# tridivb/attention_based_tbn

Hardware: AMD Instinct MI355X
Metric: clips/sec (3-seg RGB+Flow+Audio TBN fwd+bwd) (higher is better)
Workload: dtype f32; 1 GPU; BASELINE config 4: RGB+Flow+Audio async, attention off, 3 segments, 224x224 frames + 1.279 s (256x256) spectrogram, train step fwd+loss+bwd+clip+SGD; batch_per_gpu=32, global_batch=32, segments=3, parallelism=single, launch_plans=committed (bench_plans.json)

## Files before the change

attention_based_tbn_amd/_lib.py:

```python
import ctypes as C
import os

_HERE = os.path.dirname(os.path.abspath(__file__))
LIB_PATH = os.path.join(_HERE, "libtbn_hip.so")
if os.environ.get("TBN_LIB"):
    import sys as _sys
    LIB_PATH = os.path.abspath(os.environ["TBN_LIB"])
    print(f"[tbn] TBN_LIB set: loading {LIB_PATH} instead of the shipped libtbn_hip.so", file=_sys.stderr)

c_fp = C.c_void_p
c_i = C.c_int
c_sz = C.c_size_t
c_f = C.c_float


class ConvInfo(C.Structure):
    _fields_ = [("name", C.c_char * 64), ("cin", c_i), ("cout", c_i), ("ksize", c_i), ("stride", c_i),
                ("pad", c_i), ("weight_offset", c_sz), ("channel_offset", c_sz)]


class BackboneParams(C.Structure):
    _fields_ = [("weight", c_fp), ("bias", c_fp), ("gamma", c_fp), ("beta", c_fp), ("running_mean", c_fp),
                ("running_var", c_fp), ("momentum", c_f), ("eps", c_f), ("side_stream", c_fp), ("flags", c_i),
                ("weight_planes", c_fp)]
# ... 95 lines not shown
    "tbn_stem_conv_wgrad": (c_i, [c_fp, c_i, c_fp, c_fp] + [c_i] * 8 + [c_fp, c_fp]),
    "tbn_linear_fwd": (c_i, [c_fp, c_i, c_fp, c_fp, c_fp, c_i, c_i, c_i, c_i, c_i, c_fp]),
    "tbn_linear_dgrad": (c_i, [c_fp, c_i, c_fp, c_fp, c_i, c_i, c_i, c_i, c_i, c_fp, c_fp]),
    "tbn_linear_wgrad_workspace_floats": (c_sz, [c_i, c_i, c_i]),
    "tbn_linear_wgrad": (c_i, [c_fp, c_i, c_fp, c_i, c_fp, c_fp, c_i, c_i, c_i, c_fp, c_fp]),
    "tbn_bn_workspace_floats": (c_sz, [c_i, c_i]),
    "tbn_bn_relu_train_fwd": (c_i, [c_fp, c_i, c_i, c_fp, c_fp, c_fp, c_fp, c_f, c_f, c_fp, c_fp, c_fp, c_fp, c_fp,
                                    c_i, c_fp, c_fp]),
    "tbn_bn_relu_train_bwd": (c_i, [c_fp, c_i, c_fp, c_i, c_i, c_fp, c_fp, c_fp, c_fp, c_fp, c_fp, c_fp, c_fp, c_fp]),
    "tbn_bn_stats_partials": (c_i, [c_fp, c_i, c_i, c_i, c_fp, C.POINTER(c_i), c_fp]),
    "tbn_bn_fwd_batch": (c_i, [C.POINTER(BnFwdDesc), c_i, c_f, c_f, c_fp]),
    "tbn_bn_bwd_partial_floats": (c_sz, [c_i, c_i]),
    "tbn_bn_bwd_batch": (c_i, [C.POINTER(BnBwdDesc), c_i, c_fp]),
    "tbn_bn_relu_maxpool_train_fwd": (c_i, [c_fp, c_i, c_i, c_i, c_i, c_fp, c_fp, c_fp, c_fp, c_f, c_f, c_fp, c_fp, c_fp,
                                            c_fp, c_fp, c_i, c_fp, c_i, c_i, c_i, c_i, c_fp, c_fp]),
    "tbn_bn_relu_maxpool_train_bwd": (c_i, [c_fp, c_i, c_fp, c_fp, c_i, c_i, c_i, c_i, c_i, c_i, c_i, c_i, c_fp, c_fp,
                                            c_fp, c_fp, c_fp, c_fp, c_fp, c_fp, c_fp]),
    "tbn_bn_res_apply": (c_i, [c_fp, c_i, c_i, c_i, c_fp, c_fp, c_fp, c_i, c_i, c_fp, c_i, c_fp]),
    "tbn_bn_res_fwd": (c_i, [c_fp, c_i, c_i, c_i, c_fp, c_i, c_i, c_fp, c_fp, c_fp, c_fp, c_f, c_f, c_fp, c_fp, c_fp,
                             c_fp, c_fp, c_i, c_i, c_fp, c_i, c_fp]),
    "tbn_bn_res_bwd_workspace_floats": (c_sz, [c_i, c_i]),
    "tbn_bn_res_bwd": (c_i, [c_fp, c_i, c_fp, c_i, c_fp, c_i, c_i, c_i, c_fp, c_fp, c_fp, c_i, c_fp, c_i, c_fp, c_i, c_i,
                             c_fp, c_fp, c_fp, c_fp]),
    "tbn_maxpool3_fwd": (c_i, [c_fp, c_i, c_fp, c_i, c_fp] + [c_i] * 8 + [c_fp]),
    "tbn_maxpool3_bwd": (c_i, [c_fp, c_i, c_fp, c_fp, c_i] + [c_i] * 9 + [c_fp]),
    "tbn_avgpool3_fwd": (c_i, [c_fp, c_i, c_fp, c_i] + [c_i] * 5 + [c_fp]),
    "tbn_spatial_mean_fwd": (c_i, [c_fp, c_i, c_fp, c_i] + [c_i] * 5 + [c_fp]),
    "tbn_spatial_mean_bwd": (c_i, [c_fp, c_i, c_fp, c_i] + [c_i] * 5 + [c_fp]),
    "tbn_pe_concat_fwd": (c_i, [c_fp, c_i, c_fp, c_fp, c_i, c_i, c_i, c_i, c_i, c_fp]),
    "tbn_groupnorm_fwd": (c_i, [c_fp, c_fp, c_fp, c_fp, c_fp, c_fp, c_i, c_i, c_i, c_i, c_f, c_fp]),
# ... 94 lines not shown
```

attention_based_tbn_amd/core/models/bn_inception.py:

```python
import ctypes as C
import os
import weakref
from collections import OrderedDict

import torch
import torch.nn as nn

from ... import _lib
from ..._lib import BUCKET_CB, BackboneGrads, BackboneParams, ConvInfo, TbnHipError, call, lib, ptr, stream_ptr
from ... import ops

_BLOCKS = [("3a", True, True), ("3b", True, True), ("3c", False, False), ("4a", True, True), ("4b", True, True),
           ("4c", True, True), ("4d", True, True), ("4e", False, False), ("5a", True, True), ("5b", True, True)]


def reference_conv_order():
    names = ["conv1_7x7_s2", "conv2_3x3_reduce", "conv2_3x3"]
    for b, has1, hasp in _BLOCKS:
        p = "inception_" + b
        if has1:
            names.append(p + "_1x1")
        names += [p + "_3x3_reduce", p + "_3x3", p + "_double_3x3_reduce", p + "_double_3x3_1", p + "_double_3x3_2"]
        if hasp:
            names.append(p + "_pool_proj")
# ... 224 lines not shown
    def __init__(self, num_classes=1000, in_channels=3):
        super().__init__()
        self.in_channels = in_channels
        self.num_classes = num_classes
        self.is_audio = False
        self.attend = False
        self.feature_size = 1024
        self.eval_chunk = 256
        self.autotune = True
        self.use_aux_stream = True
        self._aux_streams = {}
        self.use_branch_streams = True
        self._side_streams = {}
        self.use_riders = True
        self.stem_wgrad_last = False
        self._conv_math = "f32"
        self._conv_math_layers = "3x3"
        self._planes = None
        self._planes_key = None
        self._last_flip = None
        self._out_slot = None
        self.plan_sync = None
        self.grad_bucket_fn = None
        self._plans = OrderedDict()
        probe = C.c_void_p()
        call("tbn_backbone_plan_create", in_channels, 1, 64, 64, C.byref(probe))
        self._layers = OrderedDict()
        info = ConvInfo()
        for i in range(lib().tbn_backbone_num_convs(probe)):
            call("tbn_backbone_conv_info", probe, i, C.byref(info))
# ... 108 lines not shown
        return self._plans[key]

    def plan_fingerprints(self):
        return {k: p.fingerprint() for k, p in self._plans.items()}

    def flip_weights_early(self):
        f = self._last_flip() if getattr(self, "_last_flip", None) is not None else None
        self._last_flip = None
        if f is None or f.done or f.weight._version != f.version or torch.cuda.is_current_stream_capturing():
            return False
        prm = BackboneParams(ptr(f.weight), 0, 0, 0, 0, 0, 0.1, 1e-5, 0, 0)
        call("tbn_backbone_flip_weights", f.plan.handle, C.byref(prm), ptr(f.ws), f.ws.numel(), stream_ptr())
        f.done = True
        return True

    CONV_MATH = {"f32": 0, "bf16x6": 8, "bf16x3": 16}

    @property
    def conv_math(self):
        return self._conv_math

    @conv_math.setter
    def conv_math(self, value):
        if value not in self.CONV_MATH:
            raise ValueError("conv_math must be one of %s, got %r" % (", ".join(map(repr, self.CONV_MATH)), value))
        self._conv_math = value
        if value == "f32":
            self._planes = self._planes_key = None

    CONV_MATH_LAYERS = ("3x3", "all")
# ... 18 lines not shown
        w = self.flat_weight
        np_ = 6 if self._conv_math == "bf16x6" else 3
        key = (w.data_ptr(), w._version, self._conv_math)
        nbytes = lib().tbn_backbone_weight_planes_bytes(plan.handle, np_)
        if self._planes is None or self._planes.numel() != nbytes or self._planes.device != w.device:
            self._planes, self._planes_key = torch.empty(nbytes, dtype=torch.uint8, device=w.device), None
        capturing = torch.cuda.is_current_stream_capturing()
        if self._planes_key != key or capturing:
            call("tbn_backbone_split_weights", plan.handle, ptr(w), np_, ptr(self._planes), stream_ptr())
            if not capturing:
                self._planes_key = key
        return self._planes

    def _engine_flags(self):
        return ((1 if self.use_riders else 0) | (2 if self.stem_wgrad_last else 0)
                | (0 if self.training else self.CONV_MATH[self._conv_math]) | (32 if self._planes_on() else 0))

    def _side_stream_ptr(self):
        if not self.use_branch_streams or torch.cuda.is_current_stream_capturing():
            return 0
        cur = torch.cuda.current_stream()
        s = self._side_streams.get(cur.cuda_stream)
        if s is None:
            s = self._side_streams[cur.cuda_stream] = torch.cuda.Stream(device=cur.device)
        return s.cuda_stream

    def _run(self, x, freq_only):
        if not x.is_cuda:
            raise TbnHipError("BNInception: input is on the CPU; this backbone only runs on an MI355X via "
                              "libtbn_hip.so (no CPU fallback)")
        x = x.contiguous().float()
# ... 75 lines not shown
```

attention_based_tbn_amd/csrc/api.hip:

```cpp
#include <cstdarg>
#include <cstdio>
#include <cstdlib>
#include <cstring>

#include "tbn_common.h"
#include "tbn_kernels.h"
#include "../../include/tbn_hip.h"

static thread_local char g_err[512] = "";

void tbn_set_error(const char* fmt, ...) {
  va_list ap;
  va_start(ap, fmt);
  vsnprintf(g_err, sizeof(g_err), fmt, ap);
  va_end(ap);
}

#if TBN_EXPERIMENT
int tbn_env_int(const char* name, int def, int lo, int hi) {
  const char* e = getenv(name);
  if (e == nullptr || *e == 0) return def;
  char* end = nullptr;
  const long v = strtol(e, &end, 10);
  if (end == e || *end != 0 || v < lo || v > hi) {
// ... 788 lines not shown

int tbn_bn_relu_maxpool_train_fwd(const float* y, int n, int h, int w, int c, const float* gamma, const float* beta,
                                  float* running_mean, float* running_var, float momentum, float eps, float* save_mean,
                                  float* save_rstd, float* scale, float* shift, float* pooled, int pooled_ld,
                                  uint8_t* argmax, int oh, int ow, int stride, int pad, float* workspace, void* stream) {
  hipStream_t st = (hipStream_t)stream;
  TBN_REQUIRE(y && pooled && argmax && workspace, "bn_relu_maxpool_train_fwd: null pointer");
  const int p = n * h * w;
  int parts = 0;
  TBN_TRY(tbn_launch_bn_stats(y, c, p, c, workspace, &parts, st));
  TBN_TRY(tbn_launch_bn_finalize(workspace, parts, p, c, gamma, beta, nullptr, running_mean, running_var, momentum, eps,
                                 save_mean, save_rstd, scale, shift, st));
  return tbn_launch_bn_apply_maxpool(y, n, h, w, c, scale, shift, pooled, pooled_ld, argmax, oh, ow, stride, pad, st);
}

int tbn_bn_relu_maxpool_train_bwd(const float* dpooled, int dpooled_ld, const uint8_t* argmax, const float* y, int n, int h,
                                  int w, int c, int oh, int ow, int stride, int pad, const float* save_mean,
                                  const float* save_rstd, const float* scale, const float* shift, float* dy,
                                  float* dgamma, float* dbeta, float* workspace, void* stream) {
  hipStream_t st = (hipStream_t)stream;
  TBN_REQUIRE(dpooled && argmax && y && dy && workspace, "bn_relu_maxpool_train_bwd: null pointer");
  const int p = n * h * w;
  const int parts = tbn_bn_bwd_pooled_parts(n, h, w, c, stride, pad);
  TBN_REQUIRE(parts <= tbn_bn_bwd_parts(p, c), "bn_relu_maxpool_train_bwd: workspace sized by tbn_bn_workspace_floats is too small");
  float* coef = workspace + (size_t)tbn_bn_bwd_parts(p, c) * 2 * c;
  TBN_TRY(tbn_launch_bn_bwd_reduce_pooled(dpooled, dpooled_ld, argmax, n, h, w, oh, ow, stride, pad, y, c, scale, shift,
                                          save_mean, save_rstd, workspace, st));
  TBN_TRY(tbn_launch_bn_bwd_finalize(workspace, parts, p, c, scale, save_mean, save_rstd, coef, dgamma, dbeta, nullptr, st));
  return tbn_launch_bn_bwd_apply_pooled(dpooled, dpooled_ld, argmax, n, h, w, oh, ow, stride, pad, y, c, scale, shift, coef,
                                        dy, st);
// ... 26 lines not shown
```

attention_based_tbn_amd/csrc/bn.hip:

```cpp
#include "tbn_common.h"
#include "tbn_kernels.h"
#include "tbn_bn_dev.h"
#include "tbn_pool_dev.h"

static inline int pick_chunk(int P, int rp) {
  int pch = cdiv(P, 512);
  if (pch < 64) pch = 64;
  return cdiv(pch, rp) * rp;
}

__global__ __launch_bounds__(256) void bn_stats_kernel(const float* __restrict__ y, int ld, int P, int C, int pch,
                                                       float* __restrict__ partial) {
  __shared__ float red[2 * 2048];
  const int G = C >> 2, RP = 256 / G;
  const int tid = threadIdx.x, cg = tid % G, rs = tid / G;
  const int p0 = blockIdx.x * pch, p1 = min(P, p0 + pch);
  float4 s1 = make_float4(0, 0, 0, 0), s2 = s1;
  if (rs < RP)
    for (int p = p0 + rs; p < p1; p += RP) {
      const float4 v = *reinterpret_cast<const float4*>(y + (size_t)p * ld + cg * 4);
      s1.x += v.x; s1.y += v.y; s1.z += v.z; s1.w += v.w;
      s2.x = fmaf(v.x, v.x, s2.x); s2.y = fmaf(v.y, v.y, s2.y); s2.z = fmaf(v.z, v.z, s2.z); s2.w = fmaf(v.w, v.w, s2.w);
    }
  if (rs < RP) {
// ... 125 lines not shown
  if (c < C) {
    const float sc = gamma[c] / sqrtf(var[c] + eps);
    scale[c] = sc;
    shift[c] = fmaf((bias != nullptr ? bias[c] : 0.f) - mean[c], sc, beta[c]);
  }
}

int tbn_launch_bn_fold(const float* gamma, const float* beta, const float* mean, const float* var, const float* bias,
                       float eps, float* scale, float* shift, int C, hipStream_t st) {
  TBN_KLAUNCH(bn_fold_kernel, dim3(cdiv(C, 256)), dim3(256), 0, st, gamma, beta, mean, var, bias, eps, scale,
                     shift, C);
  TBN_CHECK_LAUNCH("bn_fold");
  return TBN_OK;
}

__global__ __launch_bounds__(256) void bn_apply_maxpool_kernel(const float* __restrict__ y, int N, int H, int W, int C,
                                                               const float* __restrict__ scale,
                                                               const float* __restrict__ shift,
                                                               float* __restrict__ out, int out_ld,
                                                               unsigned char* __restrict__ argmax, int OH, int OW,
                                                               int stride, int pad, PixDecode dec) {
  const int G = C >> 2;
  const uint32_t total = (uint32_t)N * OH * OW * G;
  const unsigned nb = gridDim.x, bid = blockIdx.x;
  const unsigned q8 = nb >> 3, r8 = nb & 7, xcd = bid & 7, idx = bid >> 3;
  const uint32_t b0 = (xcd < r8 ? xcd * (q8 + 1) : r8 * (q8 + 1) + (xcd - r8) * q8) + idx;
  for (uint32_t i = b0 * 256u + threadIdx.x; i < total; i += gridDim.x * 256u) {
    int g, ox, oy, n;
    uint32_t opix;
    pix_decode(dec, i, g, ox, oy, n, opix);
    const int y0 = oy * stride - pad, x0 = ox * stride - pad;
    const float4 sc = *reinterpret_cast<const float4*>(scale + g * 4);
    const float4 sh = *reinterpret_cast<const float4*>(shift + g * 4);
    float4 best = make_float4(-INFINITY, -INFINITY, -INFINITY, -INFINITY);
    int bx = 0, by = 0, bz = 0, bw = 0;
#pragma unroll
    for (int r = 0; r < 3; ++r)
#pragma unroll
      for (int s2 = 0; s2 < 3; ++s2) {
        const int iy = y0 + r, ix = x0 + s2;
        if ((unsigned)iy < (unsigned)H && (unsigned)ix < (unsigned)W) {
          const float4 v = *reinterpret_cast<const float4*>(y + ((size_t)(n * H + iy) * W + ix) * C + g * 4);
          float4 z;
          z.x = fmaxf(fmaf(v.x, sc.x, sh.x), 0.f);
          z.y = fmaxf(fmaf(v.y, sc.y, sh.y), 0.f);
          z.z = fmaxf(fmaf(v.z, sc.z, sh.z), 0.f);
          z.w = fmaxf(fmaf(v.w, sc.w, sh.w), 0.f);
          const int k = r * 3 + s2;
          if (z.x > best.x || z.x != z.x) { best.x = z.x; bx = k; }
          if (z.y > best.y || z.y != z.y) { best.y = z.y; by = k; }
          if (z.z > best.z || z.z != z.z) { best.z = z.z; bz = k; }
          if (z.w > best.w || z.w != z.w) { best.w = z.w; bw = k; }
        }
      }
    *reinterpret_cast<float4*>(out + (size_t)opix * out_ld + g * 4) = best;
    *reinterpret_cast<uint32_t*>(argmax + (size_t)opix * C + g * 4) =
        (uint32_t)bx | ((uint32_t)by << 8) | ((uint32_t)bz << 16) | ((uint32_t)bw << 24);
  }
}

int tbn_launch_bn_apply_maxpool(const float* y, int N, int H, int W, int C, const float* scale, const float* shift,
                                float* out, int out_ld, unsigned char* argmax, int OH, int OW, int stride, int pad,
                                hipStream_t st) {
  TBN_REQUIRE(C % 4 == 0 && out_ld % 4 == 0 && argmax != nullptr, "bn_apply_maxpool: bad C / pitch / argmax");
  size_t g = ((size_t)N * OH * OW * (C / 4) + 255) / 256;
  if (g > 8192) g = 8192;
  TBN_REQUIRE((size_t)N * H * W * (C / 4) < (1ull << 31), "bn_apply_maxpool: too many elements per call");
  TBN_KLAUNCH(bn_apply_maxpool_kernel, dim3((unsigned)(g < 1 ? 1 : g)), dim3(256), 0, st, y, N, H, W, C, scale,
                     shift, out, out_ld, argmax, OH, OW, stride, pad, make_pixdecode(C / 4, OW, OH));
  TBN_CHECK_LAUNCH("bn_apply_maxpool");
  return TBN_OK;
}

struct PoolGrad {
  const float* dout;
  const unsigned char* argmax;
  int dout_ld, H, W, OH, OW, C, stride, pad;
  FastDiv div_w, div_h;
};
__device__ __forceinline__ float4 pooled_grad(const PoolGrad& q, int p, int c) {
  const uint32_t row = fdiv((uint32_t)p, q.div_w);
  const int ix = p - (int)row * q.W;
  const uint32_t n = fdiv(row, q.div_h);
  const int iy = (int)row - (int)n * q.H;
  float4 acc = make_float4(0.f, 0.f, 0.f, 0.f);
  if (q.stride == 2 && q.pad == 0) {
// ... 360 lines not shown
```

attention_based_tbn_amd/csrc/engine.hip:

```cpp
#include <string>
#include <vector>
#include <cstring>
#include <cstdio>

#include <cstdlib>
#include "tbn_common.h"
#include "tbn_kernels.h"
#include "../../include/tbn_hip.h"

namespace {

struct BlockSpec {
  const char* name;
  int cin, c1, c3r, c3, cdr, cd1, cd2;
  int pool;
  int cp, stride;
};
const BlockSpec kBlocks[] = {
    {"3a", 192, 64, 64, 64, 64, 96, 96, 0, 32, 1},     {"3b", 256, 64, 64, 96, 64, 96, 96, 0, 64, 1},
    {"3c", 320, 0, 128, 160, 64, 96, 96, 2, 0, 2},     {"4a", 576, 224, 64, 96, 96, 128, 128, 0, 128, 1},
    {"4b", 576, 192, 96, 128, 96, 128, 128, 0, 128, 1}, {"4c", 576, 160, 128, 160, 128, 160, 160, 0, 128, 1},
    {"4d", 608, 96, 128, 192, 160, 192, 192, 0, 128, 1}, {"4e", 608, 0, 128, 192, 192, 256, 256, 2, 0, 2},
    {"5a", 1056, 352, 192, 320, 160, 224, 224, 0, 128, 1}, {"5b", 1024, 352, 192, 320, 192, 224, 224, 1, 128, 1},
};
// ... 36 lines not shown
    bool pair = false;
    int p_variant = 1, p_mt = 1, p_nt = 1;
    float t = 0.f;
  } ft[2];
  int d_mt = 1, d_nt = 1, d_stages = 0;
  int d_halo = 0;
  int pair_next = -1, pair_prev = -1;
  bool pair_dgrad = false;
  int pd_variant = 1, pd_mt = 1, pd_nt = 1;
  float t_dgrad = 0.f;
  int w_mt = 0, w_nt = 0;
  bool stem;
  bool dgrad_accum;
  bool need_dgrad;
  int fuse_pool = -1;
  int nred = 0;
  int red_conv[kMaxParts], red_part[kMaxParts];
};

struct Pool {
  int kind;
  int inbuf, outbuf, out_choff, stride, pad;
  size_t argmax_off;
  bool bwd_accum;
  bool fused = false;
};

struct BnStep {
  int n;
  int conv[kMaxParts], part[kMaxParts];
// ... 405 lines not shown
      if (c.nparts == 1 && c.parts[0].dst_buf == q.inbuf && c.parts[0].dst_choff == 0 && c.cout == P->bufs[q.inbuf].C) {
        c.fuse_pool = (int)pi;
        q.fused = true;
      }
  }

  for (size_t ci = 0; ci < P->convs.size(); ++ci) {
    Conv& f = P->convs[ci];
    if (!f.need_dgrad || last_conv[f.inbuf] != (int)ci || f.inbuf == P->out_buf) continue;
    struct Cand { int conv, part, choff; };
    std::vector<Cand> cand;
    bool ok = true;
    for (size_t cj = 0; cj < P->convs.size(); ++cj) {
      const Conv& c = P->convs[cj];
      for (int k = 0; k < c.nparts; ++k)
        if (c.parts[k].dst_buf == f.inbuf) {
          if (c.fuse_pool >= 0) ok = false;
          cand.push_back({(int)cj, k, c.parts[k].dst_choff});
        }
    }
    if (!ok || cand.empty() || (int)cand.size() > kMaxParts) continue;
    for (size_t a = 0; a < cand.size(); ++a)
      for (size_t b = a + 1; b < cand.size(); ++b)
        if (cand[b].choff < cand[a].choff) std::swap(cand[a], cand[b]);
    for (auto& cd : cand)
      if (cd.choff % 32 != 0) ok = false;
    if (!ok) continue;
    f.nred = (int)cand.size();
    for (int k = 0; k < f.nred; ++k) {
      f.red_conv[k] = cand[k].conv;
      f.red_part[k] = cand[k].part;
      P->convs[cand[k].conv].parts[cand[k].part].red_src = (int)ci;
    }
  }
  return true;
}

#ifndef TBN_DIAG
#define TBN_DIAG 0
#endif
static inline bool diag_skip(int bit) {
// ... 68 lines not shown
  for (auto& c : P->convs)
    for (int k = 0; k < c.nparts; ++k)
      if (c.parts[k].pooled) {
        c.parts[k].yraw_off = take(R * c.outH * c.outW * c.parts[k].cout);
        c.parts[k].y2_off = take(R * c.outH * c.outW * c.parts[k].cout);
      }
  P->eval_floats = off;
  for (auto& c : P->convs) c.y_off = take(R * c.outH * c.outW * c.cout);
  for (size_t i = 1; i < P->bufs.size(); ++i) {
    if ((int)i == P->out_buf) continue;
    P->bufs[i].doff = take(R * P->bufs[i].H * P->bufs[i].W * P->bufs[i].C);
  }
  for (auto& c : P->convs)
    for (int k = 0; k < c.nparts; ++k)
      if (c.parts[k].red_src >= 0) {
        const Buf& db = P->bufs[c.parts[k].dst_buf];
        const int drows = (int)(R * db.H * db.W);
        c.parts[k].bpart_off = take(((size_t)cdiv(drows, drows <= kSk4MaxRows ? 32 : 128) + 4) * 2 * c.parts[k].cout);
      }
  P->coef_off = take(TBN_BN_MAXL * 3 * 1024);
  P->diag_fold_off = take(2 * 2048);
  P->wsplit_off = take(wsplit);
  P->wt_off = take(wtf);
  P->dwpack_off = take((size_t)64 * P->stem_rows * P->kw);
  size_t bytes = off * sizeof(float);
  P->argmax_bytes_off = bytes;
  for (auto& p : P->pools)
    if (p.kind == 1) {
      const Buf& ob = P->bufs[p.outbuf];
      const Buf& ib = P->bufs[p.inbuf];
      p.argmax_off = bytes;
      bytes += align_up(R * ob.H * ob.W * ib.C, 256);
    }
// ... 367 lines not shown
  const Conv::FwdTune& T = c.ft[gemm];
  return {T.halo, T.mt, T.pair, T.p_mt};
}
int pair_role(const tbn_backbone_plan* P, const Conv& c, int gemm, bool br) {
  if (br) return 0;
  if (c.pair_next >= 0 && tuned(c, gemm).pair) return 1;
  if (c.pair_prev >= 0 && tuned(P->convs[c.pair_prev], gemm).pair) return 2;
  return 0;
}
int writer_rows(const tbn_backbone_plan* P, const Conv& c, int gemm, bool br) {
  const int role = pair_role(P, c, gemm, br);
  if (role == 0) return tile_rows(tuned(c, gemm).halo, tuned(c, gemm).mt);
  return 128 * tuned(role == 1 ? c : P->convs[c.pair_prev], gemm).p_mt;
}

void fill_dgrad(const tbn_backbone_plan* P, const Conv& c, float* ws, int R, ConvP* pp) {
  ConvP& p = *pp;
  const Buf& ib = P->bufs[c.inbuf];
  memset(&p, 0, sizeof(p));
  p.in = ws + c.y_off;
  p.in_ld = c.cout;
  p.wt = ws + P->wt_off + c.w_off;
  p.N = R;
  p.H = c.outH;
  p.W = c.outW;
  p.OH = c.inH;
  p.OW = c.inW;
  p.Cin = c.cout;
  p.Cout = c.cin;
  p.R = p.S = c.k;
  p.stride = 1;
  p.pad = c.k - 1 - c.pad;
// ... 10 lines not shown
  p.stages = c.d_stages;
  p.halo = c.d_halo;
  p.nred = c.nred;
  p.red_chan = (int)P->chan_floats;
  for (int k = 0; k < c.nred; ++k) {
    const Conv& pc = P->convs[c.red_conv[k]];
    const Part& q = pc.parts[c.red_part[k]];
    RedSeg& r = p.red[k];
    r.y = q.pooled ? ws + q.y2_off : ws + pc.y_off + q.col0;
    r.y_ld = q.pooled ? q.cout : pc.cout;
    r.partial = ws + q.bpart_off;
    r.stats = ws + P->stats_off;
    r.col_begin = q.dst_choff;
    r.C = q.cout;
    r.c_off = (int)q.c_off;
  }
  if (c.nred > 0 && p.red[0].col_begin != 0) {
    p.nred = 0;
  }
}

void fill_wgrad(const tbn_backbone_plan* P, const Conv& c, float* ws, int R, WgradP* wp) {
  const Buf& ib = P->bufs[c.inbuf];
  memset(wp, 0, sizeof(*wp));
  wp->dy = ws + c.y_off;
  wp->dy_ld = c.cout;
  wp->x = ws + ib.off;
  wp->x_ld = ib.C;
  wp->N = R;
  wp->H = c.inH;
  wp->W = c.inW;
// ... 247 lines not shown
            TBN_TRY(tbn_launch_bn_apply(ws + q.y2_off, R * c.outH * c.outW, q.cout, scale + q.c_off, shift + q.c_off, &z, 1, st));
        }
        continue;
      }
      const Conv& c0 = P->convs[s.conv[0]];
      if (s.n == 1 && c0.fuse_pool >= 0) {
        const Part& q = c0.parts[0];
        const int M = R * c0.outH * c0.outW;
        const Pool& pl = P->pools[c0.fuse_pool];
        const Buf& ob = P->bufs[pl.outbuf];
        if (!diag_skip(2)) {
          TBN_TRY(tbn_launch_bn_finalize(ws + P->partial_off + (size_t)c0.slot * P->partial_floats, cdiv(M, writer_rows(P, c0, GEMM_FWD_TRAIN, br)), M,
                                         q.cout, prm->gamma + q.c_off, prm->beta + q.c_off, prm->bias + q.c_off,
                                         prm->running_mean + q.c_off, prm->running_var + q.c_off, prm->momentum, prm->eps,
                                         mean + q.c_off, rstd + q.c_off, scale + q.c_off, shift + q.c_off, st));
          TBN_TRY(tbn_launch_bn_apply_maxpool(ws + c0.y_off, (int)R, c0.outH, c0.outW, q.cout, scale + q.c_off,
                                              shift + q.c_off, ws + ob.off + pl.out_choff, ob.C,
                                              (uint8_t*)workspace + pl.argmax_off, ob.H, ob.W, pl.stride, pl.pad, st));
        }
        continue;
      }
      BnFwdBatch fb;
      memset(&fb, 0, sizeof(fb));
      fb.n = s.n;
      fb.momentum = prm->momentum;
      fb.eps = prm->eps;
      for (int k = 0; k < s.n; ++k) {
        const Conv& c = P->convs[s.conv[k]];
        const Part& q = c.parts[s.part[k]];
        const Buf& db = P->bufs[q.dst_buf];
        const int M = R * c.outH * c.outW;
        BnFwdLayer& L = fb.l[k];
        L.P = M;
// ... 327 lines not shown
  float* coef = ws + P->coef_off;
  auto dptr = [&](int buf) -> const float* {
    return buf == P->out_buf ? dfeatures : ws + P->bufs[buf].doff;
  };

  if ((prm->flags & TBN_BACKBONE_WEIGHTS_FLIPPED) == 0)
    TBN_TRY(tbn_launch_weight_flip_transpose_all(prm->weight, ws + P->wt_off, P->flip, st));
  const std::vector<Op>& prog = br ? P->ops_b : P->ops;
  const hipStream_t st_main = st;
  const bool use_riders = !br && (prm->flags & TBN_BACKBONE_RIDERS) != 0 && !tbn_prof_enabled() && !P->riders.empty();
  RiderP bpend;
  int bpend_host = -1;
  PM->rider_launches[1] = 0;
  int deferred[8], ndef = 0;
  const bool stem_last = !br && aux == nullptr && (prm->flags & TBN_BACKBONE_STEM_WGRAD_LAST) != 0;
  auto issue_wgrad = [&](const Conv& c, hipStream_t wst) -> int {
    tbn_prof_label(("wgrad " + c.parts[c.nparts - 1].name).c_str());
    WgradP wp;
    fill_wgrad(P, c, ws, R, &wp);
    if (c.stem) {
      float* dwp = ws + P->dwpack_off;
      TBN_TRY(tbn_launch_wgrad(wp, 1, dwp, ws + P->wsplit_off, wst));
      if (P->stem_mode == 1) return tbn_launch_unpack_stem_wgrad_rows(dwp, g->dweight + c.w_off, 64, P->cin0, P->kw, wst);
      return tbn_launch_unpack_stem_wgrad_s2d(dwp, g->dweight + c.w_off, 64, P->cin0, wst);
    }
    return tbn_launch_wgrad(wp, 0, g->dweight + c.w_off, ws + P->wsplit_off, wst);
  };
  const int* blk_op = br ? P->block_op_b : P->block_op;
  size_t bucket_hi = P->weight_floats;
  auto fire_bucket = [&](int blk) -> int {
// ... 45 lines not shown
      continue;
    }
    if (o.kind == OP_BN) {
      const BnStep& s = P->bns[o.idx];
      const Conv& c0 = P->convs[s.conv[0]];
      if (s.n == 1 && c0.fuse_pool >= 0) {
        const Part& q = c0.parts[0];
        const int M = R * c0.outH * c0.outW;
        const Pool& pl = P->pools[c0.fuse_pool];
        const Buf& ob = P->bufs[pl.outbuf];
        const float* dpool = dptr(pl.outbuf) + pl.out_choff;
        const uint8_t* am = (const uint8_t*)workspace + pl.argmax_off;
        float* y = ws + c0.y_off;
        const bool bn_grad = g->dgamma && g->dbeta && (g->bn_grad_layers == 2 || (g->bn_grad_layers == 1 && s.conv[0] == 0));
        if (!diag_skip(8)) {
          TBN_TRY(tbn_launch_bn_bwd_reduce_pooled(dpool, ob.C, am, R, c0.outH, c0.outW, ob.H, ob.W, pl.stride, pl.pad, y,
                                                  q.cout, scale + q.c_off, shift + q.c_off, mean + q.c_off,
                                                  rstd + q.c_off, partial, st));
          TBN_TRY(tbn_launch_bn_bwd_finalize(partial, tbn_bn_bwd_pooled_parts(R, c0.outH, c0.outW, q.cout, pl.stride, pl.pad), M,
                                             q.cout, scale + q.c_off,
                                             mean + q.c_off, rstd + q.c_off, coef, bn_grad ? g->dgamma + q.c_off : nullptr,
                                             bn_grad ? g->dbeta + q.c_off : nullptr, g->dbias + q.c_off, st));
          TBN_TRY(tbn_launch_bn_bwd_apply_pooled(dpool, ob.C, am, R, c0.outH, c0.outW, ob.H, ob.W, pl.stride, pl.pad, y,
                                                 q.cout, scale + q.c_off, shift + q.c_off, coef, y, st));
        }
        continue;
      }
      auto fill_layer = [&](BnBwdLayer& L, int ci, int pk, int slot) {
        const Conv& c = P->convs[ci];
        const Part& q = c.parts[pk];
        const Buf& db = P->bufs[q.dst_buf];
        L.nseg = 1;
        L.dz[0].ptr = dptr(q.dst_buf) + q.dst_choff;
        L.dz[0].ld = db.C;
// ... 57 lines not shown
      TBN_TRY(issue_wgrad(c, aux));
    } else if (br && o.side) {
      TBN_REQUIRE(ndef < 8, "backbone_backward: too many deferred weight gradients");
      deferred[ndef++] = o.idx;
    } else if (stem_last && (o.idx == 1 || o.idx == 2)) {
      deferred[ndef++] = o.idx;
    } else {
      TBN_TRY(issue_wgrad(c, st));
    }
    if (c.need_dgrad) {
      const int role = pair_role(P, c, GEMM_DGRAD, br);
      if (role == 2) continue;
      if (role == 1) {
        const Conv& c2 = P->convs[c.pair_next];
        ConvP pa, pb;
        fill_dgrad(P, c, ws, R, &pa);
        fill_dgrad(P, c2, ws, R, &pb);
        tbn_prof_label(("dgrad " + c.parts[0].name + " | " + c2.parts[0].name).c_str());
        TBN_TRY(tbn_launch_conv_pair(pa, pb, c.pd_variant, c.pd_mt, c.pd_nt, st));
        continue;
      }
      tbn_prof_label(("dgrad " + c.parts[c.nparts - 1].name).c_str());
      ConvP p;
      fill_dgrad(P, c, ws, R, &p);
      const RiderP* rd = (bpend_host == o.idx) ? &bpend : nullptr;
      if (rd != nullptr) {
        bpend_host = -1;
        ++PM->rider_launches[1];
      }
      TBN_TRY(tbn_launch_conv(p, 0, c.d_mt, c.d_nt, st, rd));
    }
  }
  if (stem_last) {
    for (int k = 0; k < ndef; ++k) TBN_TRY(issue_wgrad(P->convs[deferred[k]], st_main));
    ndef = 0;
  }
  TBN_REQUIRE(bpend_host < 0, "backbone_backward: a rider was left without its host launch (conv %d)", bpend_host);
  return TBN_OK;
}
// ... 3 lines not shown
```

attention_based_tbn_amd/csrc/tbn_kernels.h:

```cpp
#pragma once
#include "tbn_common.h"
#include <hip/hip_ext.h>
#include <type_traits>

enum { CONV_EPI_PLAIN = 0, CONV_EPI_STATS = 1, CONV_EPI_EVAL = 2 };
enum {
  CONV_FLAG_ACCUM = 1,
  CONV_FLAG_RELU = 2,
  CONV_FLAG_HALO = 4,
  CONV_FLAG_DMA = 8,
  CONV_FLAG_SK4 = 16,
  CONV_FLAG_BF16X6 = 32,
  CONV_FLAG_BF16X3 = 64,
  CONV_FLAG_BF16X_PLANES = 128,
  CONV_FLAG_DESC_OUT2 = 256
};

#define TBN_CONV_MAXSEG 4
struct RedSeg {
  const float* y;
  float* partial;
  const float* stats;
  int y_ld, col_begin, C, c_off;
  unsigned y_bytes;
// ... 213 lines not shown
  short cout[64], cin[64], taps[64];
  int blk0[65];
};
int tbn_launch_weight_flip_transpose_all(const float* w, float* wt, const FlipTab& tab, hipStream_t st);

int tbn_launch_bn_stats(const float* y, int ld, int P, int C, float* partial, int* nparts, hipStream_t st);
int tbn_bn_stats_parts(int P, int C);
int tbn_launch_bn_finalize(const float* partial, int nparts, int P, int C, const float* gamma, const float* beta,
                           const float* conv_bias, float* running_mean, float* running_var, float momentum, float eps,
                           float* save_mean, float* save_rstd, float* scale, float* shift, hipStream_t st);
int tbn_launch_bn_apply(const float* y, int P, int C, const float* scale, const float* shift, const Seg* segs,
                        int nseg, hipStream_t st);
int tbn_launch_bn_apply_maxpool(const float* y, int N, int H, int W, int C, const float* scale, const float* shift,
                                float* out, int out_ld, unsigned char* argmax, int OH, int OW, int stride, int pad,
                                hipStream_t st);
int tbn_launch_bn_bwd_reduce_pooled(const float* dpooled, int dpooled_ld, const unsigned char* argmax, int N, int H,
                                    int W, int OH, int OW, int stride, int pad, const float* y, int C,
                                    const float* scale, const float* shift, const float* mean, const float* rstd,
                                    float* partial, hipStream_t st);
int tbn_bn_bwd_pooled_parts(int N, int H, int W, int C, int stride, int pad);
int tbn_launch_bn_bwd_apply_pooled(const float* dpooled, int dpooled_ld, const unsigned char* argmax, int N, int H, int W,
                                   int OH, int OW, int stride, int pad, const float* y, int C, const float* scale,
                                   const float* shift, const float* coef, float* dy, hipStream_t st);
#define TBN_BN_MAXL 4
struct BnFwdLayer {
  const float* y;
  int y_ld;
  int P, C;
  const float* partial;
  int pld, nparts;
// ... 65 lines not shown
```

include/tbn_hip.h:

```cpp
#ifndef TBN_HIP_H
#define TBN_HIP_H
#include <stddef.h>
#include <stdint.h>
#ifdef __cplusplus
extern "C" {
#endif

#define TBN_ERR_ARG (-1)
#define TBN_ERR_LAUNCH (-2)
#define TBN_ERR_UNSUPPORTED (-3)

int tbn_version(void);
#define TBN_CAP_CONV_BF16X 1
#define TBN_CAP_CONV_BF16X_PLANES 2
#define TBN_CAP_FRAMES_CROPS 4
#define TBN_CAP_ATTN_GENERAL 8
#define TBN_CAP_ATTN_REG 16
#define TBN_CAP_AUDIO_LAYER 32
#define TBN_CAP_STEM_OPS 64
#define TBN_CAP_BN_BATCH_OPS 128
int tbn_capabilities(void);
const char* tbn_last_error(void);

int tbn_profile_enable(int on);
// ... 19 lines not shown
  const float* beta;
  float* running_mean;
  float* running_var;
  float momentum;
  float eps;
  void* side_stream;
  int flags;
  const void* weight_planes;
} tbn_backbone_params;
#define TBN_BACKBONE_RIDERS 1
#define TBN_BACKBONE_STEM_WGRAD_LAST 2
#define TBN_BACKBONE_WEIGHTS_FLIPPED 4
#define TBN_BACKBONE_CONV_BF16X6 8
#define TBN_BACKBONE_CONV_BF16X3 16
#define TBN_BACKBONE_CONV_BF16X_ALL 32

typedef struct {
  float* dweight;
  float* dbias;
  float* dgamma;
  float* dbeta;
  int bn_grad_layers;
  void* aux_stream;
  void (*bucket_cb)(void* user, size_t first_float, size_t num_floats);
  void* bucket_user;
} tbn_backbone_grads;

int tbn_backbone_plan_create(int in_channels, int frames, int height, int width, tbn_backbone_plan** plan);
void tbn_backbone_plan_destroy(tbn_backbone_plan* plan);
int tbn_backbone_num_convs(const tbn_backbone_plan* plan);
// ... 96 lines not shown
int tbn_linear_wgrad(const float* dy, int dy_ld, const float* x, int x_ld, float* dw, float* dbias, int m, int k,
                     int n, float* workspace, void* stream);

size_t tbn_bn_workspace_floats(int p, int c);
int tbn_bn_relu_train_fwd(const float* y, int p, int c, const float* gamma, const float* beta, float* running_mean,
                          float* running_var, float momentum, float eps, float* save_mean, float* save_rstd,
                          float* scale, float* shift, float* z, int z_ld, float* workspace, void* stream);
int tbn_bn_relu_train_bwd(const float* dz, int dz_ld, const float* y, int p, int c, const float* save_mean,
                          const float* save_rstd, const float* scale, const float* shift, float* dy, float* dgamma,
                          float* dbeta, float* workspace, void* stream);

int tbn_bn_relu_maxpool_train_fwd(const float* y, int n, int h, int w, int c, const float* gamma, const float* beta,
                                  float* running_mean, float* running_var, float momentum, float eps, float* save_mean,
                                  float* save_rstd, float* scale, float* shift, float* pooled, int pooled_ld,
                                  uint8_t* argmax, int oh, int ow, int stride, int pad, float* workspace, void* stream);
int tbn_bn_relu_maxpool_train_bwd(const float* dpooled, int dpooled_ld, const uint8_t* argmax, const float* y, int n, int h,
                                  int w, int c, int oh, int ow, int stride, int pad, const float* save_mean,
                                  const float* save_rstd, const float* scale, const float* shift, float* dy,
                                  float* dgamma, float* dbeta, float* workspace, void* stream);

typedef struct {
  float* ptr;
  int ld;
  int col_begin;
} tbn_bn_seg;
typedef struct {
  const float* y;
  int y_ld;
  int p, c;
  const float* partial;
// ... 154 lines not shown
```

Measured before the change: 894.5 clips/s.

## Fuse stem BN-backward reduction into downstream dgrad via kept pre-pool values

The stem's fused BN+ReLU+maxpool forward now also stores the pre-activation value of the pooled argmax winner. The consumer conv's dgrad reduction rider can then compute the BN backward partial sums for the pooled stem layer directly. This removes the separate bn_bwd_reduce_pooled pass over the full-resolution stem activation. The cost is extra workspace and an extra write of pooled-size data in forward, plus a flag to fall back to the old path.

```diff
diff --git a/attention_based_tbn_amd/_lib.py b/attention_based_tbn_amd/_lib.py
--- a/attention_based_tbn_amd/_lib.py
+++ b/attention_based_tbn_amd/_lib.py
@@ -133,6 +133,8 @@
     "tbn_bn_bwd_batch": (c_i, [C.POINTER(BnBwdDesc), c_i, c_fp]),
     "tbn_bn_relu_maxpool_train_fwd": (c_i, [c_fp, c_i, c_i, c_i, c_i, c_fp, c_fp, c_fp, c_fp, c_f, c_f, c_fp, c_fp, c_fp,
                                             c_fp, c_fp, c_i, c_fp, c_i, c_i, c_i, c_i, c_fp, c_fp]),
+    "tbn_bn_relu_maxpool_keep_train_fwd": (c_i, [c_fp, c_i, c_i, c_i, c_i, c_fp, c_fp, c_fp, c_fp, c_f, c_f, c_fp, c_fp,
+                                                 c_fp, c_fp, c_fp, c_i, c_fp, c_fp, c_i, c_i, c_i, c_i, c_i, c_fp, c_fp]),
     "tbn_bn_relu_maxpool_train_bwd": (c_i, [c_fp, c_i, c_fp, c_fp, c_i, c_i, c_i, c_i, c_i, c_i, c_i, c_i, c_fp, c_fp,
                                             c_fp, c_fp, c_fp, c_fp, c_fp, c_fp, c_fp]),
     "tbn_bn_res_apply": (c_i, [c_fp, c_i, c_i, c_i, c_fp, c_fp, c_fp, c_i, c_i, c_fp, c_i, c_fp]),
diff --git a/attention_based_tbn_amd/core/models/bn_inception.py b/attention_based_tbn_amd/core/models/bn_inception.py
--- a/attention_based_tbn_amd/core/models/bn_inception.py
+++ b/attention_based_tbn_amd/core/models/bn_inception.py
@@ -262,6 +262,7 @@
         self._side_streams = {}
         self.use_riders = True
         self.stem_wgrad_last = False
+        self.stem_red = True
         self._conv_math = "f32"
         self._conv_math_layers = "3x3"
         self._planes = None
@@ -400,6 +401,7 @@
         f.done = True
         return True
 
+    STEM_REDUCE_PASS = 64
     CONV_MATH = {"f32": 0, "bf16x6": 8, "bf16x3": 16}
 
     @property
@@ -448,7 +450,8 @@
 
     def _engine_flags(self):
         return ((1 if self.use_riders else 0) | (2 if self.stem_wgrad_last else 0)
-                | (0 if self.training else self.CONV_MATH[self._conv_math]) | (32 if self._planes_on() else 0))
+                | (0 if self.training else self.CONV_MATH[self._conv_math]) | (32 if self._planes_on() else 0)
+                | (0 if self.stem_red else self.STEM_REDUCE_PASS))
 
     def _side_stream_ptr(self):
         if not self.use_branch_streams or torch.cuda.is_current_stream_capturing():
diff --git a/attention_based_tbn_amd/csrc/api.hip b/attention_based_tbn_amd/csrc/api.hip
--- a/attention_based_tbn_amd/csrc/api.hip
+++ b/attention_based_tbn_amd/csrc/api.hip
@@ -826,6 +826,22 @@
   return tbn_launch_bn_apply_maxpool(y, n, h, w, c, scale, shift, pooled, pooled_ld, argmax, oh, ow, stride, pad, st);
 }
 
+int tbn_bn_relu_maxpool_keep_train_fwd(const float* y, int n, int h, int w, int c, const float* gamma, const float* beta,
+                                       float* running_mean, float* running_var, float momentum, float eps,
+                                       float* save_mean, float* save_rstd, float* scale, float* shift, float* pooled,
+                                       int pooled_ld, uint8_t* argmax, float* yp, int yp_ld, int oh, int ow, int stride,
+                                       int pad, float* workspace, void* stream) {
+  hipStream_t st = (hipStream_t)stream;
+  TBN_REQUIRE(y && pooled && argmax && yp && workspace, "bn_relu_maxpool_keep_train_fwd: null pointer");
+  const int p = n * h * w;
+  int parts = 0;
+  TBN_TRY(tbn_launch_bn_stats(y, c, p, c, workspace, &parts, st));
+  TBN_TRY(tbn_launch_bn_finalize(workspace, parts, p, c, gamma, beta, nullptr, running_mean, running_var, momentum, eps,
+                                 save_mean, save_rstd, scale, shift, st));
+  return tbn_launch_bn_apply_maxpool_keep(y, n, h, w, c, scale, shift, pooled, pooled_ld, argmax, yp, yp_ld, oh, ow, stride,
+                                          pad, st);
+}
+
 int tbn_bn_relu_maxpool_train_bwd(const float* dpooled, int dpooled_ld, const uint8_t* argmax, const float* y, int n, int h,
                                   int w, int c, int oh, int ow, int stride, int pad, const float* save_mean,
                                   const float* save_rstd, const float* scale, const float* shift, float* dy,
diff --git a/attention_based_tbn_amd/csrc/bn.hip b/attention_based_tbn_amd/csrc/bn.hip
--- a/attention_based_tbn_amd/csrc/bn.hip
+++ b/attention_based_tbn_amd/csrc/bn.hip
@@ -163,12 +163,14 @@
   return TBN_OK;
 }
 
+template <bool KEEP>
 __global__ __launch_bounds__(256) void bn_apply_maxpool_kernel(const float* __restrict__ y, int N, int H, int W, int C,
                                                                const float* __restrict__ scale,
                                                                const float* __restrict__ shift,
                                                                float* __restrict__ out, int out_ld,
                                                                unsigned char* __restrict__ argmax, int OH, int OW,
-                                                               int stride, int pad, PixDecode dec) {
+                                                               int stride, int pad, PixDecode dec,
+                                                               float* __restrict__ yp, int yp_ld) {
   const int G = C >> 2;
   const uint32_t total = (uint32_t)N * OH * OW * G;
   const unsigned nb = gridDim.x, bid = blockIdx.x;
@@ -183,6 +185,7 @@
     const float4 sh = *reinterpret_cast<const float4*>(shift + g * 4);
     float4 best = make_float4(-INFINITY, -INFINITY, -INFINITY, -INFINITY);
     int bx = 0, by = 0, bz = 0, bw = 0;
+    float4 yb = make_float4(0.f, 0.f, 0.f, 0.f);
 #pragma unroll
     for (int r = 0; r < 3; ++r)
 #pragma unroll
@@ -196,29 +199,43 @@
           z.z = fmaxf(fmaf(v.z, sc.z, sh.z), 0.f);
           z.w = fmaxf(fmaf(v.w, sc.w, sh.w), 0.f);
           const int k = r * 3 + s2;
-          if (z.x > best.x || z.x != z.x) { best.x = z.x; bx = k; }
-          if (z.y > best.y || z.y != z.y) { best.y = z.y; by = k; }
-          if (z.z > best.z || z.z != z.z) { best.z = z.z; bz = k; }
-          if (z.w > best.w || z.w != z.w) { best.w = z.w; bw = k; }
+          if (z.x > best.x || z.x != z.x) { best.x = z.x; bx = k; if (KEEP) yb.x = v.x; }
+          if (z.y > best.y || z.y != z.y) { best.y = z.y; by = k; if (KEEP) yb.y = v.y; }
+          if (z.z > best.z || z.z != z.z) { best.z = z.z; bz = k; if (KEEP) yb.z = v.z; }
+          if (z.w > best.w || z.w != z.w) { best.w = z.w; bw = k; if (KEEP) yb.w = v.w; }
         }
       }
     *reinterpret_cast<float4*>(out + (size_t)opix * out_ld + g * 4) = best;
+    if (KEEP) tbn_st4<(TBN_BN_NT & 16) != 0>(yp + (size_t)opix * yp_ld + g * 4, yb);
     *reinterpret_cast<uint32_t*>(argmax + (size_t)opix * C + g * 4) =
         (uint32_t)bx | ((uint32_t)by << 8) | ((uint32_t)bz << 16) | ((uint32_t)bw << 24);
   }
+}
+
+int tbn_launch_bn_apply_maxpool_keep(const float* y, int N, int H, int W, int C, const float* scale, const float* shift,
+                                     float* out, int out_ld, unsigned char* argmax, float* yp, int yp_ld, int OH, int OW,
+                                     int stride, int pad, hipStream_t st) {
+  TBN_REQUIRE(C % 4 == 0 && out_ld % 4 == 0 && argmax != nullptr, "bn_apply_maxpool: bad C / pitch / argmax");
+  TBN_REQUIRE(yp == nullptr || (yp_ld % 4 == 0 && yp_ld >= C), "bn_apply_maxpool: bad yp pitch %d", yp_ld);
+  size_t g = ((size_t)N * OH * OW * (C / 4) + 255) / 256;
+  if (g > 8192) g = 8192;
+  TBN_REQUIRE((size_t)N * H * W * (C / 4) < (1ull << 31), "bn_apply_maxpool: too many elements per call");
+  const dim3 grid((unsigned)(g < 1 ? 1 : g));
+  if (yp != nullptr) {
+    TBN_KLAUNCH(bn_apply_maxpool_kernel<true>, grid, dim3(256), 0, st, y, N, H, W, C, scale, shift, out, out_ld, argmax,
+                       OH, OW, stride, pad, make_pixdecode(C / 4, OW, OH), yp, yp_ld);
+  } else {
+    TBN_KLAUNCH(bn_apply_maxpool_kernel<false>, grid, dim3(256), 0, st, y, N, H, W, C, scale, shift, out, out_ld, argmax,
+                       OH, OW, stride, pad, make_pixdecode(C / 4, OW, OH), yp, yp_ld);
+  }
+  TBN_CHECK_LAUNCH("bn_apply_maxpool");
+  return TBN_OK;
 }
 
 int tbn_launch_bn_apply_maxpool(const float* y, int N, int H, int W, int C, const float* scale, const float* shift,
                                 float* out, int out_ld, unsigned char* argmax, int OH, int OW, int stride, int pad,
                                 hipStream_t st) {
-  TBN_REQUIRE(C % 4 == 0 && out_ld % 4 == 0 && argmax != nullptr, "bn_apply_maxpool: bad C / pitch / argmax");
-  size_t g = ((size_t)N * OH * OW * (C / 4) + 255) / 256;
-  if (g > 8192) g = 8192;
-  TBN_REQUIRE((size_t)N * H * W * (C / 4) < (1ull << 31), "bn_apply_maxpool: too many elements per call");
-  TBN_KLAUNCH(bn_apply_maxpool_kernel, dim3((unsigned)(g < 1 ? 1 : g)), dim3(256), 0, st, y, N, H, W, C, scale,
-                     shift, out, out_ld, argmax, OH, OW, stride, pad, make_pixdecode(C / 4, OW, OH));
-  TBN_CHECK_LAUNCH("bn_apply_maxpool");
-  return TBN_OK;
+  return tbn_launch_bn_apply_maxpool_keep(y, N, H, W, C, scale, shift, out, out_ld, argmax, nullptr, 0, OH, OW, stride, pad, st);
 }
 
 struct PoolGrad {
diff --git a/attention_based_tbn_amd/csrc/engine.hip b/attention_based_tbn_amd/csrc/engine.hip
--- a/attention_based_tbn_amd/csrc/engine.hip
+++ b/attention_based_tbn_amd/csrc/engine.hip
@@ -74,6 +74,7 @@
   bool dgrad_accum;
   bool need_dgrad;
   int fuse_pool = -1;
+  size_t yp_off = 0;
   int nred = 0;
   int red_conv[kMaxParts], red_part[kMaxParts];
 };
@@ -509,10 +510,8 @@
     for (size_t cj = 0; cj < P->convs.size(); ++cj) {
       const Conv& c = P->convs[cj];
       for (int k = 0; k < c.nparts; ++k)
-        if (c.parts[k].dst_buf == f.inbuf) {
-          if (c.fuse_pool >= 0) ok = false;
-          cand.push_back({(int)cj, k, c.parts[k].dst_choff});
-        }
+        if (c.parts[k].dst_buf == f.inbuf) cand.push_back({(int)cj, k, c.parts[k].dst_choff});
+      if (c.fuse_pool >= 0 && P->pools[c.fuse_pool].outbuf == f.inbuf) cand.push_back({(int)cj, 0, P->pools[c.fuse_pool].out_choff});
     }
     if (!ok || cand.empty() || (int)cand.size() > kMaxParts) continue;
     for (size_t a = 0; a < cand.size(); ++a)
@@ -520,6 +519,7 @@
         if (cand[b].choff < cand[a].choff) std::swap(cand[a], cand[b]);
     for (auto& cd : cand)
       if (cd.choff % 32 != 0) ok = false;
+    if (cand[0].choff != 0) ok = false;
     if (!ok) continue;
     f.nred = (int)cand.size();
     for (int k = 0; k < f.nred; ++k) {
@@ -618,9 +618,10 @@
   for (auto& c : P->convs)
     for (int k = 0; k < c.nparts; ++k)
       if (c.parts[k].red_src >= 0) {
-        const Buf& db = P->bufs[c.parts[k].dst_buf];
+        const Buf& db = P->bufs[c.fuse_pool >= 0 ? P->pools[c.fuse_pool].outbuf : c.parts[k].dst_buf];
         const int drows = (int)(R * db.H * db.W);
         c.parts[k].bpart_off = take(((size_t)cdiv(drows, drows <= kSk4MaxRows ? 32 : 128) + 4) * 2 * c.parts[k].cout);
+        if (c.fuse_pool >= 0) c.yp_off = take((size_t)drows * c.cout);
       }
   P->coef_off = take(TBN_BN_MAXL * 3 * 1024);
   P->diag_fold_off = take(2 * 2048);
@@ -1018,8 +1019,9 @@
   return 128 * tuned(role == 1 ? c : P->convs[c.pair_prev], gemm).p_mt;
 }
 
-void fill_dgrad(const tbn_backbone_plan* P, const Conv& c, float* ws, int R, ConvP* pp) {
+void fill_dgrad(const tbn_backbone_plan* P, const Conv& c, float* ws, int R, ConvP* pp, bool stem_red = true) {
   ConvP& p = *pp;
+  bool any_y = false;
   const Buf& ib = P->bufs[c.inbuf];
   memset(&p, 0, sizeof(p));
   p.in = ws + c.y_off;
@@ -1060,7 +1062,16 @@
     r.col_begin = q.dst_choff;
     r.C = q.cout;
     r.c_off = (int)q.c_off;
-  }
+    if (pc.fuse_pool >= 0) {
+      r.y = stem_red ? ws + pc.yp_off : nullptr;
+      r.y_ld = pc.cout;
+      r.col_begin = P->pools[pc.fuse_pool].out_choff;
+      any_y = any_y || stem_red;
+    } else {
+      any_y = true;
+    }
+  }
+  if (!any_y) p.nred = 0;
   if (c.nred > 0 && p.red[0].col_begin != 0) {
     p.nred = 0;
   }
@@ -1338,9 +1349,11 @@
                                          q.cout, prm->gamma + q.c_off, prm->beta + q.c_off, prm->bias + q.c_off,
                                          prm->running_mean + q.c_off, prm->running_var + q.c_off, prm->momentum, prm->eps,
                                          mean + q.c_off, rstd + q.c_off, scale + q.c_off, shift + q.c_off, st));
-          TBN_TRY(tbn_launch_bn_apply_maxpool(ws + c0.y_off, (int)R, c0.outH, c0.outW, q.cout, scale + q.c_off,
-                                              shift + q.c_off, ws + ob.off + pl.out_choff, ob.C,
-                                              (uint8_t*)workspace + pl.argmax_off, ob.H, ob.W, pl.stride, pl.pad, st));
+          TBN_TRY(tbn_launch_bn_apply_maxpool_keep(ws + c0.y_off, (int)R, c0.outH, c0.outW, q.cout, scale + q.c_off,
+                                                   shift + q.c_off, ws + ob.off + pl.out_choff, ob.C,
+                                                   (uint8_t*)workspace + pl.argmax_off,
+                                                   q.red_src >= 0 ? ws + c0.yp_off : nullptr, q.cout, ob.H, ob.W, pl.stride,
+                                                   pl.pad, st));
         }
         continue;
       }
@@ -1698,6 +1711,7 @@
   PM->rider_launches[1] = 0;
   int deferred[8], ndef = 0;
   const bool stem_last = !br && aux == nullptr && (prm->flags & TBN_BACKBONE_STEM_WGRAD_LAST) != 0;
+  const bool stem_red = (prm->flags & TBN_BACKBONE_STEM_REDUCE_PASS) == 0;
   auto issue_wgrad = [&](const Conv& c, hipStream_t wst) -> int {
     tbn_prof_label(("wgrad " + c.parts[c.nparts - 1].name).c_str());
     WgradP wp;
@@ -1773,10 +1787,19 @@
         float* y = ws + c0.y_off;
         const bool bn_grad = g->dgamma && g->dbeta && (g->bn_grad_layers == 2 || (g->bn_grad_layers == 1 && s.conv[0] == 0));
         if (!diag_skip(8)) {
-          TBN_TRY(tbn_launch_bn_bwd_reduce_pooled(dpool, ob.C, am, R, c0.outH, c0.outW, ob.H, ob.W, pl.stride, pl.pad, y,
-                                                  q.cout, scale + q.c_off, shift + q.c_off, mean + q.c_off,
-                                                  rstd + q.c_off, partial, st));
-          TBN_TRY(tbn_launch_bn_bwd_finalize(partial, tbn_bn_bwd_pooled_parts(R, c0.outH, c0.outW, q.cout, pl.stride, pl.pad), M,
+          const float* parts = partial;
+          int nparts;
+          if (stem_red && q.red_src >= 0) {
+            const Conv& f = P->convs[q.red_src];
+            parts = ws + q.bpart_off;
+            nparts = tbn_conv_red_rows(R, f.inH, f.inW, f.stride, writer_rows(P, f, GEMM_DGRAD, br));
+          } else {
+            TBN_TRY(tbn_launch_bn_bwd_reduce_pooled(dpool, ob.C, am, R, c0.outH, c0.outW, ob.H, ob.W, pl.stride, pl.pad, y,
+                                                    q.cout, scale + q.c_off, shift + q.c_off, mean + q.c_off,
+                                                    rstd + q.c_off, partial, st));
+            nparts = tbn_bn_bwd_pooled_parts(R, c0.outH, c0.outW, q.cout, pl.stride, pl.pad);
+          }
+          TBN_TRY(tbn_launch_bn_bwd_finalize(parts, nparts, M,
                                              q.cout, scale + q.c_off,
                                              mean + q.c_off, rstd + q.c_off, coef, bn_grad ? g->dgamma + q.c_off : nullptr,
                                              bn_grad ? g->dbeta + q.c_off : nullptr, g->dbias + q.c_off, st));
@@ -1864,15 +1887,15 @@
       if (role == 1) {
         const Conv& c2 = P->convs[c.pair_next];
         ConvP pa, pb;
-        fill_dgrad(P, c, ws, R, &pa);
-        fill_dgrad(P, c2, ws, R, &pb);
+        fill_dgrad(P, c, ws, R, &pa, stem_red);
+        fill_dgrad(P, c2, ws, R, &pb, stem_red);
         tbn_prof_label(("dgrad " + c.parts[0].name + " | " + c2.parts[0].name).c_str());
         TBN_TRY(tbn_launch_conv_pair(pa, pb, c.pd_variant, c.pd_mt, c.pd_nt, st));
         continue;
       }
       tbn_prof_label(("dgrad " + c.parts[c.nparts - 1].name).c_str());
       ConvP p;
-      fill_dgrad(P, c, ws, R, &p);
+      fill_dgrad(P, c, ws, R, &p, stem_red);
       const RiderP* rd = (bpend_host == o.idx) ? &bpend : nullptr;
       if (rd != nullptr) {
         bpend_host = -1;
diff --git a/attention_based_tbn_amd/csrc/tbn_kernels.h b/attention_based_tbn_amd/csrc/tbn_kernels.h
--- a/attention_based_tbn_amd/csrc/tbn_kernels.h
+++ b/attention_based_tbn_amd/csrc/tbn_kernels.h
@@ -251,6 +251,9 @@
 int tbn_launch_bn_apply_maxpool(const float* y, int N, int H, int W, int C, const float* scale, const float* shift,
                                 float* out, int out_ld, unsigned char* argmax, int OH, int OW, int stride, int pad,
                                 hipStream_t st);
+int tbn_launch_bn_apply_maxpool_keep(const float* y, int N, int H, int W, int C, const float* scale, const float* shift,
+                                     float* out, int out_ld, unsigned char* argmax, float* yp, int yp_ld, int OH, int OW,
+                                     int stride, int pad, hipStream_t st);
 int tbn_launch_bn_bwd_reduce_pooled(const float* dpooled, int dpooled_ld, const unsigned char* argmax, int N, int H,
                                     int W, int OH, int OW, int stride, int pad, const float* y, int C,
                                     const float* scale, const float* shift, const float* mean, const float* rstd,
diff --git a/include/tbn_hip.h b/include/tbn_hip.h
--- a/include/tbn_hip.h
+++ b/include/tbn_hip.h
@@ -57,6 +57,7 @@
 #define TBN_BACKBONE_CONV_BF16X6 8
 #define TBN_BACKBONE_CONV_BF16X3 16
 #define TBN_BACKBONE_CONV_BF16X_ALL 32
+#define TBN_BACKBONE_STEM_REDUCE_PASS 64
 
 typedef struct {
   float* dweight;
@@ -183,6 +184,11 @@
                                   float* running_mean, float* running_var, float momentum, float eps, float* save_mean,
                                   float* save_rstd, float* scale, float* shift, float* pooled, int pooled_ld,
                                   uint8_t* argmax, int oh, int ow, int stride, int pad, float* workspace, void* stream);
+int tbn_bn_relu_maxpool_keep_train_fwd(const float* y, int n, int h, int w, int c, const float* gamma, const float* beta,
+                                       float* running_mean, float* running_var, float momentum, float eps,
+                                       float* save_mean, float* save_rstd, float* scale, float* shift, float* pooled,
+                                       int pooled_ld, uint8_t* argmax, float* yp, int yp_ld, int oh, int ow, int stride,
+                                       int pad, float* workspace, void* stream);
 int tbn_bn_relu_maxpool_train_bwd(const float* dpooled, int dpooled_ld, const uint8_t* argmax, const float* y, int n, int h,
                                   int w, int c, int oh, int ow, int stride, int pad, const float* save_mean,
                                   const float* save_rstd, const float* scale, const float* shift, float* dy,
```

After: 900.3 clips/s, median of 6. About the same (+0.7%).
